# safaad/aim

Hardware: AMD Instinct MI355X
Metric: aligned pairs/sec WFA-adaptive l=100 e=1% (higher is better)
Workload: dtype int16

## Files before the change

aim_amd/csrc/wfa_lane.hpp:

```cpp
#pragma once

#include <utility>

#include "aim_device.hpp"

#ifndef AIM_LANE_MIN_WAVES
#define AIM_LANE_MIN_WAVES 1
#endif
#ifndef AIM_LANE_FULLWAIT
#define AIM_LANE_FULLWAIT 0
#endif
#ifndef AIM_LANE_INTERLEAVE
#define AIM_LANE_INTERLEAVE 2
#endif
#ifndef AIM_LANE_SPREAD_PCT
#define AIM_LANE_SPREAD_PCT 67
#endif
#ifndef AIM_LANE_ASM_ROWS
#define AIM_LANE_ASM_ROWS 1
#endif
#ifndef AIM_LANE_NT_STORE
#define AIM_LANE_NT_STORE 0
#endif
#ifndef AIM_LANE_PACK_X2
#define AIM_LANE_PACK_X2 0
#endif
#ifndef AIM_LANE_STAMPS
#define AIM_LANE_STAMPS 0
#endif
#ifndef AIM_LANE_DIAG
#define AIM_LANE_DIAG 0
#endif
#ifndef AIM_LANE_RES_STAGE
#define AIM_LANE_RES_STAGE 1
#endif
#ifndef AIM_LANE_DMA_AUX
#define AIM_LANE_DMA_AUX 2
#endif
#ifndef AIM_LANE_WGS_PER_CU
#define AIM_LANE_WGS_PER_CU 8
#endif
#if AIM_LANE_STAMPS
#define AIM_STAMP(i) do { unsigned long long t_; __builtin_amdgcn_sched_barrier(0); \
        asm volatile("s_memtime %0\n\ts_waitcnt lgkmcnt(0)" : "=s"(t_) :: "memory"); __builtin_amdgcn_sched_barrier(0); \
        stamp_sum[i] += t_ - stamp_last; stamp_last = t_; } while (0)
#else
#define AIM_STAMP(i) do { } while (0)
#endif

namespace aim {

constexpr int kLaneNull = -16384;

template <int X, int O, int E, int MAXS>
struct WfShape {
    bool present[MAXS + 1];
    bool hasI[MAXS + 1];
    bool hasD[MAXS + 1];
    int lo[MAXS + 1];
    int hi[MAXS + 1];
    int kmin, kmax, maxw;
    constexpr WfShape() : present{}, hasI{}, hasD{}, lo{}, hi{}, kmin(0), kmax(0), maxw(1)
    {
        present[0] = true;
        for (int s = 1; s <= MAXS; ++s) {
            const int ss = s - X, so = s - O - E, se = s - E;
            const bool m_sub_null = ss < 0 || !present[ss];
            const bool m_o_null = so < 0 || !present[so];
            const bool i_e_null = se < 0 || !present[se] || !hasI[se];
            const bool d_e_null = se < 0 || !present[se] || !hasD[se];
            const bool i_out_null = m_o_null && i_e_null;
            const bool d_out_null = m_o_null && d_e_null;
            if (m_sub_null && i_out_null && d_out_null) continue;
            const int sub_lo = m_sub_null ? 1 : lo[ss], sub_hi = m_sub_null ? -1 : hi[ss];
            const int o_lo = m_o_null ? 1 : lo[so], o_hi = m_o_null ? -1 : hi[so];
            const bool e_none = i_e_null && d_e_null;
            const int e_lo = e_none ? 1 : lo[se], e_hi = e_none ? -1 : hi[se];
            int l = sub_lo < o_lo ? sub_lo : o_lo;
            l = (l < e_lo ? l : e_lo) - 1;
            int h = sub_hi > o_hi ? sub_hi : o_hi;
            h = (h > e_hi ? h : e_hi) + 1;
            present[s] = true;
            hasI[s] = !i_out_null;
            hasD[s] = !d_out_null;
            lo[s] = l;
            hi[s] = h;
            if (l < kmin) kmin = l;
            if (h > kmax) kmax = h;
            if (h - l + 1 > maxw) maxw = h - l + 1;
        }
    }
};

template <int X, int O, int E, int MAXS>
struct WfHist {
    int m[MAXS + 1], i[MAXS + 1], d[MAXS + 1];
    int meta, total;
    constexpr WfHist() : m{}, i{}, d{}, meta(0), total(0)
    {
        constexpr WfShape<X, O, E, MAXS> SH{};
        int at = 0;
        for (int s = 0; s <= MAXS; ++s) {
            const int w = SH.present[s] ? SH.hi[s] - SH.lo[s] + 1 : 0;
            m[s] = at; at += w;
            i[s] = at; at += (SH.present[s] && SH.hasI[s]) ? w : 0;
            d[s] = at; at += (SH.present[s] && SH.hasD[s]) ? w : 0;
        }
        meta = at;
        total = at + 3 * (MAXS + 1);
    }
};
enum { LF_PRESENT = 1, LF_MNULL = 2, LF_INULL = 4, LF_DNULL = 8, LF_HASI = 16, LF_HASD = 32 };

template <int NP>
__device__ __forceinline__ int first_stop(const uint32_t (&m)[NP], int v)
{
    const int wi = v >> 4;
    const uint32_t lowmask = ~0u << ((v & 15) * 2);
    int res = NP * 16;
#pragma unroll
    for (int j = NP - 1; j >= 0; --j) {
        uint32_t mj = m[j];
        mj = (j == wi) ? (mj & lowmask) : mj;
        mj = (j < wi) ? 0u : mj;
        const int pos = j * 16 + (__builtin_ctz(mj | 0x80000000u) >> 1);
        res = mj ? pos : res;
    }
    return res;
}

typedef __attribute__((address_space(3))) void *lds_ptr_t;
__device__ __forceinline__ lds_ptr_t lds_at(uint32_t byte_off) { return (lds_ptr_t)(uintptr_t)byte_off; }

template <int... I>
__device__ __forceinline__ void dma_full_pieces(uint32_t lds_off, const char *g_lane, std::integer_sequence<int, I...>)
{
    (__builtin_amdgcn_global_load_lds((const __attribute__((address_space(1))) void *)(g_lane + (I >> 2) * 4096),
                                      lds_at(lds_off + (I >> 2) * 4096), 16, (I & 3) * 1024, AIM_LANE_DMA_AUX), ...);
}

template <int I>
__device__ __forceinline__ void dma_piece(uint32_t lds_off, const char *g_lane)
{
    __builtin_amdgcn_global_load_lds((const __attribute__((address_space(1))) void *)(g_lane + (I >> 2) * 4096),
                                      lds_at(lds_off + (I >> 2) * 4096), 16, (I & 3) * 1024, AIM_LANE_DMA_AUX);
    __builtin_amdgcn_sched_barrier(0);
}

template <int X, int O, int E, int MAXS, int NP, int PCT>
struct LaneSpread {
    int cells, last;
    constexpr LaneSpread() : cells(0), last(0)
    {
        constexpr WfShape<X, O, E, MAXS> SH{};
        for (int s = 0; s <= MAXS; ++s) cells += SH.present[s] ? SH.hi[s] - SH.lo[s] + 1 : 0;
        const int c = (cells * PCT + 99) / 100;
        last = NP + 1 + (c < 1 ? 1 : c);
    }
    constexpr int due(int slot) const { return slot >= last ? NP + 1 : (slot * (NP + 1)) / last; }
};

template <typename F, int... I>
__device__ __forceinline__ void lane_pieces(int from, int to, F &f, std::integer_sequence<int, I...>)
{
    ((I >= from && I < to ? f(std::integral_constant<int, I>{}) : void()), ...);
}
template <int N, typename F>
__device__ __forceinline__ void lane_pieces_from(int first, F &f)
{
    static_assert(N <= 8, "one case per piece");
    switch (first) {
    case 0: if constexpr (0 < N) f(std::integral_constant<int, 0>{}); [[fallthrough]];
    case 1: if constexpr (1 < N) f(std::integral_constant<int, 1>{}); [[fallthrough]];
    case 2: if constexpr (2 < N) f(std::integral_constant<int, 2>{}); [[fallthrough]];
    case 3: if constexpr (3 < N) f(std::integral_constant<int, 3>{}); [[fallthrough]];
    case 4: if constexpr (4 < N) f(std::integral_constant<int, 4>{}); [[fallthrough]];
    case 5: if constexpr (5 < N) f(std::integral_constant<int, 5>{}); [[fallthrough]];
    case 6: if constexpr (6 < N) f(std::integral_constant<int, 6>{}); [[fallthrough]];
    case 7: if constexpr (7 < N) f(std::integral_constant<int, 7>{}); [[fallthrough]];
    default: break;
    }
}

template <int RS, int NCH>
__device__ __forceinline__ void dma_rows(uint32_t lds_off, const char *base, uint32_t pair0, uint32_t n_pairs, int lane)
{
    const char *g = base + (uint64_t)pair0 * RS;
    if (pair0 + kWave <= n_pairs) {
        dma_full_pieces(lds_off, g + (uint32_t)lane * 16u, std::make_integer_sequence<int, NCH>{});
    } else {
        const uint32_t rows = n_pairs - pair0;
        const uint32_t n_chunks = (rows * RS + 15) / 16;
#pragma unroll
        for (int i = 0; i < NCH; ++i) {
            const uint32_t c = i * kWave + lane;
            if (c < n_chunks)
                __builtin_amdgcn_global_load_lds((const __attribute__((address_space(1))) void *)(g + (uint64_t)c * 16),
                                                 lds_at(lds_off + i * kWave * 16), 16, 0, AIM_LANE_DMA_AUX);
        }
    }
}

__device__ __forceinline__ void stage_requests(uint32_t lds_off, const KArgs &a, uint32_t pair0, int lane)
{
    const uint32_t rqb = (a.p.flags & AIM_FLAG_REQ8) ? 8u : 16u;
    const char *g = reinterpret_cast<const char *>(a.req) + (uint64_t)pair0 * rqb;
    if (pair0 + kWave <= a.n_pairs) {
        if ((uint32_t)lane * 16u < kWave * rqb)
            __builtin_amdgcn_global_load_lds((const __attribute__((address_space(1))) void *)(g + (uint64_t)lane * 16),
                                             lds_at(lds_off), 16, 0, 0);
    } else {
        const uint32_t n_dw = (a.n_pairs - pair0) * (rqb / 4u);
#pragma unroll
        for (int i = 0; i < 4; ++i) {
            const uint32_t c = i * kWave + lane;
            if (c < n_dw)
                __builtin_amdgcn_global_load_lds((const __attribute__((address_space(1))) void *)(g + (uint64_t)c * 4),
                                                 lds_at(lds_off + i * kWave * 4), 4, 0, 0);
        }
    }
}

typedef uint32_t lane_u32x4 __attribute__((ext_vector_type(4)));
typedef uint32_t lane_u32x2 __attribute__((ext_vector_type(2)));

struct LaneReqAddr { uint32_t lo, hi; };
__device__ __forceinline__ LaneReqAddr staged_request_addr(uint32_t lds_req_off, const KArgs &a, int lane)
{
    const bool r8 = a.p.flags & AIM_FLAG_REQ8;
    LaneReqAddr q;
    q.lo = lds_req_off + (uint32_t)lane * (r8 ? 8u : 16u);
    q.hi = q.lo + (r8 ? 4u : 12u);
    return q;
}
__device__ __forceinline__ aim_request_t decode_staged_request(const lane_u32x2 &lo, uint32_t hi, const KArgs &a)
{
    aim_request_t r;
    r.padding = 0; r.idx = hi;
    if (a.p.flags & AIM_FLAG_REQ8) { r.pattern_len = (int16_t)(lo.x & 0xffffu); r.text_len = (int16_t)(lo.x >> 16); }
    else { r.pattern_len = (int)lo.x; r.text_len = (int)lo.y; }
    return r;
}

template <int RS, int NP>
__device__ __forceinline__ void read_group(const LaneReqAddr &qa, uint32_t row_addr, lane_u32x2 &q_lo, uint32_t &q_hi,
                                           lane_u32x4 (&P)[NP], lane_u32x4 (&T)[NP])
{
    static_assert(NP == 5 || NP == 7, "READ_SIZE 80 or 112");
#if AIM_LANE_ASM_ROWS
    if constexpr (NP == 7) {
        asm volatile("ds_read_b64 %0, %[qlo]\n\tds_read_b32 %1, %[qhi]\n\t"
                     "ds_read_b128 %2, %[row]\n\tds_read_b128 %3, %[row] offset:16\n\tds_read_b128 %4, %[row] offset:32\n\t"
                     "ds_read_b128 %5, %[row] offset:48\n\tds_read_b128 %6, %[row] offset:64\n\tds_read_b128 %7, %[row] offset:80\n\t"
                     "ds_read_b128 %8, %[row] offset:96\n\t"
                     "ds_read_b128 %9, %[row] offset:%c[tb]\n\tds_read_b128 %10, %[row] offset:%c[tb]+16\n\tds_read_b128 %11, %[row] offset:%c[tb]+32\n\t"
                     "ds_read_b128 %12, %[row] offset:%c[tb]+48\n\tds_read_b128 %13, %[row] offset:%c[tb]+64\n\tds_read_b128 %14, %[row] offset:%c[tb]+80\n\t"
                     "ds_read_b128 %15, %[row] offset:%c[tb]+96\n\t"
                     "s_waitcnt lgkmcnt(0)"
                     : "=&v"(q_lo), "=&v"(q_hi), "=&v"(P[0]), "=&v"(P[1]), "=&v"(P[2]), "=&v"(P[3]), "=&v"(P[4]), "=&v"(P[5]), "=&v"(P[6]),
                       "=&v"(T[0]), "=&v"(T[1]), "=&v"(T[2]), "=&v"(T[3]), "=&v"(T[4]), "=&v"(T[5]), "=&v"(T[6])
                     : [qlo] "v"(qa.lo), [qhi] "v"(qa.hi), [row] "v"(row_addr), [tb] "n"(kWave * RS)
                     : "memory");
    } else {
        asm volatile("ds_read_b64 %0, %[qlo]\n\tds_read_b32 %1, %[qhi]\n\t"
                     "ds_read_b128 %2, %[row]\n\tds_read_b128 %3, %[row] offset:16\n\tds_read_b128 %4, %[row] offset:32\n\t"
                     "ds_read_b128 %5, %[row] offset:48\n\tds_read_b128 %6, %[row] offset:64\n\t"
                     "ds_read_b128 %7, %[row] offset:%c[tb]\n\tds_read_b128 %8, %[row] offset:%c[tb]+16\n\tds_read_b128 %9, %[row] offset:%c[tb]+32\n\t"
                     "ds_read_b128 %10, %[row] offset:%c[tb]+48\n\tds_read_b128 %11, %[row] offset:%c[tb]+64\n\t"
                     "s_waitcnt lgkmcnt(0)"
                     : "=&v"(q_lo), "=&v"(q_hi), "=&v"(P[0]), "=&v"(P[1]), "=&v"(P[2]), "=&v"(P[3]), "=&v"(P[4]),
                       "=&v"(T[0]), "=&v"(T[1]), "=&v"(T[2]), "=&v"(T[3]), "=&v"(T[4])
                     : [qlo] "v"(qa.lo), [qhi] "v"(qa.hi), [row] "v"(row_addr), [tb] "n"(kWave * RS)
                     : "memory");
    }
#else
    typedef const __attribute__((address_space(3))) lane_u32x4 *lds_row_t;
    q_lo = *reinterpret_cast<const __attribute__((address_space(3))) lane_u32x2 *>((uintptr_t)qa.lo);
    q_hi = *reinterpret_cast<const __attribute__((address_space(3))) uint32_t *>((uintptr_t)qa.hi);
#pragma unroll
    for (int j = 0; j < NP; ++j) P[j] = reinterpret_cast<lds_row_t>((uintptr_t)row_addr)[j];
#pragma unroll
    for (int j = 0; j < NP; ++j) T[j] = reinterpret_cast<lds_row_t>((uintptr_t)(row_addr + kWave * RS))[j];
    asm volatile("s_waitcnt lgkmcnt(0)" ::: "memory");
#endif
}

template <int J, bool MASKED, int NP, typename StepF>
__device__ __forceinline__ void pack_step(const lane_u32x4 (&raw)[NP], int len, uint32_t (&out)[NP], uint32_t &bad, StepF &after_step)
{
    const uint32_t a[4] = {raw[J].x, raw[J].y, raw[J].z, raw[J].w};
    uint32_t b[4];
#if AIM_LANE_PACK_X2
#pragma unroll
    for (int i = 0; i < 4; ++i) {
        const uint32_t t2 = a[i] & 0x06060606u;
        const uint32_t rec = __builtin_amdgcn_perm(0x00470054u, 0x00430041u, t2);
        if (MASKED) {
            const int rem = len - 4 * (4 * J + i);
            const uint32_t mask = rem >= 4 ? ~0u : (rem <= 0 ? 0u : ((1u << (8 * rem)) - 1u));
            bad |= (rec ^ a[i]) & mask;
        } else {
            bad = __builtin_amdgcn_sad_u8(rec, a[i], bad);
        }
        b[i] = __builtin_amdgcn_udot4(t2, 0x40100401u, 0u, false);
    }
    out[J] = ((b[0] | (b[1] << 8) | (b[2] << 16)) >> 1) | (b[3] << 23);
#else
#pragma unroll
    for (int i = 0; i < 4; ++i) {
        const uint32_t t = (a[i] >> 1) & 0x03030303u;
        const uint32_t rec = __builtin_amdgcn_perm(0u, 0x47544341u, t);
        if (MASKED) {
            const int rem = len - 4 * (4 * J + i);
            const uint32_t mask = rem >= 4 ? ~0u : (rem <= 0 ? 0u : ((1u << (8 * rem)) - 1u));
            bad |= (rec ^ a[i]) & mask;
        } else {
            bad = __builtin_amdgcn_sad_u8(rec, a[i], bad);
        }
        b[i] = __builtin_amdgcn_udot4(t, 0x40100401u, 0u, false);
    }
    out[J] = b[0] | (b[1] << 8) | (b[2] << 16) | (b[3] << 24);
#endif
    after_step(std::integral_constant<int, J>{});
}
template <bool FAST, int NP, typename StepF, int... J>
__device__ __forceinline__ uint32_t pack_row_seq(const lane_u32x4 (&raw)[NP], int len, uint32_t (&out)[NP], StepF &after_step,
                                                 std::integer_sequence<int, J...>)
{
    uint32_t bad = 0;
    (pack_step<J, (!FAST || J == NP - 1), NP>(raw, len, out, bad, after_step), ...);
    return bad;
}
template <bool FAST, int NP, typename StepF>
__device__ __forceinline__ uint32_t pack_row(const lane_u32x4 (&raw)[NP], int len, uint32_t (&out)[NP], StepF after_step)
{
    return pack_row_seq<FAST, NP>(raw, len, out, after_step, std::make_integer_sequence<int, NP>{});
}

enum : uint32_t { LANE_TODO_COUNT = 0, LANE_TODO_LIST = 16 };

template <int NP>
__device__ __forceinline__ void raw_diag(const lane_u32x4 (&rawP)[NP], const lane_u32x4 (&rawT)[NP], int k, uint32_t (&out)[NP])
{
    uint32_t pw[4 * NP], tw[4 * NP];
#pragma unroll
    for (int j = 0; j < NP; ++j) {
        pw[4 * j] = rawP[j].x; pw[4 * j + 1] = rawP[j].y; pw[4 * j + 2] = rawP[j].z; pw[4 * j + 3] = rawP[j].w;
        tw[4 * j] = rawT[j].x; tw[4 * j + 1] = rawT[j].y; tw[4 * j + 2] = rawT[j].z; tw[4 * j + 3] = rawT[j].w;
    }
#pragma unroll
    for (int j = 0; j < NP; ++j) {
        uint32_t b[4];
#pragma unroll
        for (int i = 0; i < 4; ++i) {
            const int w = 4 * j + i;
            const int o = 4 * w + k;
            const int wi = (o >= 0) ? (o >> 2) : -((-o + 3) >> 2);
            const int sh = o - 4 * wi;
            const uint32_t lo = (wi >= 0 && wi < 4 * NP) ? tw[wi] : 0u;
            const uint32_t hi = (wi + 1 >= 0 && wi + 1 < 4 * NP) ? tw[wi + 1] : 0u;
            const uint32_t ts = sh ? __builtin_amdgcn_alignbyte(hi, lo, (uint32_t)sh) : lo;
            const uint32_t x = pw[w] ^ ts;
            const uint32_t nz = ((((x & 0x7f7f7f7fu) + 0x7f7f7f7fu) | x) >> 7) & 0x01010101u;
            b[i] = __builtin_amdgcn_udot4(nz, 0x40100401u, 0u, false);
        }
        out[j] = b[0] | (b[1] << 8) | (b[2] << 16) | (b[3] << 24);
    }
}



struct LaneNoCell { __device__ __forceinline__ void operator()() const {} };
template <int X, int O, int E, int MAXS, int NP, int KW, bool HIST = false, typename CellF = LaneNoCell>
__device__ __forceinline__ int wfa_scores_dynamic(const uint32_t (&dk)[KW][NP], int plen, int tlen, int ms_run, bool reduce, bool active,
                                                  int16_t *hist = nullptr, CellF on_cell = CellF{})
{
    constexpr WfShape<X, O, E, MAXS> SH{};
    constexpr WfHist<X, O, E, MAXS> HX{};
    bool hasi[MAXS + 1], hasd[MAXS + 1];
    static_assert(KW == SH.kmax - SH.kmin + 1, "diagonal window");
    static_assert(SH.kmax < 16 && SH.kmin > -16, "diagonal shifts are single-word funnel shifts");
    const int ak = tlen - plen;
    int Mv[MAXS + 1][KW], Iv[MAXS + 1][KW], Dv[MAXS + 1][KW];
    int klo[MAXS + 1], khi[MAXS + 1];
    bool pres[MAXS + 1], mnul[MAXS + 1], inul[MAXS + 1], dnul[MAXS + 1];
    int score = MAXS + 1;
    bool done = false;
#pragma unroll
    for (int s = 0; s <= MAXS; ++s) {
        if (!SH.present[s]) {
            pres[s] = false; mnul[s] = inul[s] = dnul[s] = true; klo[s] = 0; khi[s] = -1; hasi[s] = hasd[s] = false;
            if (HIST) { hist[(HX.meta + 3 * s) * kWave] = 0; hist[(HX.meta + 3 * s + 1) * kWave] = -1; hist[(HX.meta + 3 * s + 2) * kWave] = 0; }
            continue;
        }
        if (s == 0) {
            pres[0] = true; mnul[0] = false; inul[0] = dnul[0] = true; klo[0] = khi[0] = 0; hasi[0] = hasd[0] = false;
            Mv[0][-SH.kmin] = 0;
        } else {
            const int ss = s - X, so = s - O - E, se = s - E;
            const bool m_sub_null = ss < 0 || !SH.present[ss] || !pres[ss < 0 ? 0 : ss] || mnul[ss < 0 ? 0 : ss];
            const bool m_o_null = so < 0 || !SH.present[so] || !pres[so < 0 ? 0 : so] || mnul[so < 0 ? 0 : so];
            const bool i_e_null = se < 0 || !SH.present[se] || !pres[se < 0 ? 0 : se] || inul[se < 0 ? 0 : se];
            const bool d_e_null = se < 0 || !SH.present[se] || !pres[se < 0 ? 0 : se] || dnul[se < 0 ? 0 : se];
            const bool i_out_null = m_o_null && i_e_null, d_out_null = m_o_null && d_e_null;
            pres[s] = !(m_sub_null && i_out_null && d_out_null);
            const int sub_lo = m_sub_null ? 1 : klo[ss < 0 ? 0 : ss], sub_hi = m_sub_null ? -1 : khi[ss < 0 ? 0 : ss];
            const int o_lo = m_o_null ? 1 : klo[so < 0 ? 0 : so], o_hi = m_o_null ? -1 : khi[so < 0 ? 0 : so];
            const bool e_none = i_e_null && d_e_null;
            const int e_lo = e_none ? 1 : klo[se < 0 ? 0 : se], e_hi = e_none ? -1 : khi[se < 0 ? 0 : se];
            klo[s] = min(min(sub_lo, o_lo), e_lo) - 1;
            khi[s] = max(max(sub_hi, o_hi), e_hi) + 1;
            mnul[s] = false; inul[s] = i_out_null; dnul[s] = d_out_null;
            hasi[s] = !i_out_null; hasd[s] = !d_out_null;
#pragma unroll
            for (int k = SH.lo[s]; k <= SH.hi[s]; ++k) {
                const int kk = k - SH.kmin;
                const int km1 = kk > 0 ? kk - 1 : 0, kp1 = kk + 1 < KW ? kk + 1 : KW - 1;
                const int sso = so < 0 ? 0 : so, sse = se < 0 ? 0 : se, sss = ss < 0 ? 0 : ss;
                int ins = -10;
                {
                    const int ins_g = (!m_o_null && o_lo <= k - 1 && k - 1 <= o_hi) ? Mv[sso][km1] : kLaneNull;
                    const int ins_i = (!i_e_null && e_lo <= k - 1 && k - 1 <= e_hi) ? Iv[sse][km1] : kLaneNull;
                    const int v = (ins_g == kLaneNull && ins_i == kLaneNull) ? kLaneNull : max(ins_g, ins_i) + 1;
                    ins = i_out_null ? -10 : v;
                    Iv[s][kk] = v;
                    if (HIST && SH.hasI[s]) hist[(HX.i[s] + k - SH.lo[s]) * kWave] = (int16_t)v;
                }
                int del = -10;
                {
                    const int del_g = (!m_o_null && o_lo <= k + 1 && k + 1 <= o_hi) ? Mv[sso][kp1] : kLaneNull;
                    const int del_d = (!d_e_null && e_lo <= k + 1 && k + 1 <= e_hi) ? Dv[sse][kp1] : kLaneNull;
                    const int v = max(del_g, del_d);
                    del = d_out_null ? -10 : v;
                    Dv[s][kk] = v;
                    if (HIST && SH.hasD[s]) hist[(HX.d[s] + k - SH.lo[s]) * kWave] = (int16_t)v;
                }
                int sub = -10;
                if (!m_sub_null) sub = (sub_lo <= k && k <= sub_hi) ? Mv[sss][kk] + 1 : kLaneNull;
                Mv[s][kk] = max(del, max(sub, ins));
            }
        }
#pragma unroll
        for (int k = SH.lo[s]; k <= SH.hi[s]; ++k) {
            const int kk = k - SH.kmin;
            int off = Mv[s][kk];
            const int v = off - k;
            const int limit = min(plen, tlen - k);
            if (off >= 0 && v >= 0 && v < limit) {
                const int stop = min(first_stop<NP>(dk[kk], v), limit);
                off += stop - v;
            }
            Mv[s][kk] = off;
            if (HIST) hist[(HX.m[s] + k - SH.lo[s]) * kWave] = (int16_t)off;
            on_cell();
        }
        if (SH.hi[s] - SH.lo[s] + 1 >= 10) {
            const bool apply = reduce && pres[s] && !mnul[s] && (khi[s] - klo[s] + 1) >= 10;
            int dist[KW];
            int min_distance = max(plen, tlen);
#pragma unroll
            for (int k = SH.lo[s]; k <= SH.hi[s]; ++k) {
                const int kk = k - SH.kmin;
                const int off = Mv[s][kk];
                dist[kk] = max(plen - (off - k), tlen - off);
                if (klo[s] <= k && k <= khi[s]) min_distance = min(min_distance, dist[kk]);
            }
            int kfirst = 0x7fffffff, klast = -0x7fffffff;
#pragma unroll
            for (int k = SH.lo[s]; k <= SH.hi[s]; ++k) {
                const int kk = k - SH.kmin;
                const bool ok = klo[s] <= k && k <= khi[s] && (dist[kk] - min_distance) <= 50;
                kfirst = ok ? min(kfirst, k) : kfirst;
                klast = ok ? max(klast, k) : klast;
            }
            int nklo = klo[s], nkhi = khi[s];
            const int top_limit = min(ak - 1, khi[s]);
            if (klo[s] < top_limit) nklo = min(top_limit, kfirst);
            const int bottom_limit = max(ak + 1, nklo);
            if (khi[s] > bottom_limit) nkhi = max(bottom_limit, klast);
            const bool kill = nklo > nkhi;
            if (apply) {
                mnul[s] = kill; inul[s] = inul[s] || kill; dnul[s] = dnul[s] || kill;
                klo[s] = kill ? klo[s] : nklo;
                khi[s] = kill ? khi[s] : nkhi;
            }
        }
        if (HIST) {
            hist[(HX.meta + 3 * s) * kWave] = (int16_t)klo[s];
            hist[(HX.meta + 3 * s + 1) * kWave] = (int16_t)khi[s];
            hist[(HX.meta + 3 * s + 2) * kWave] = (int16_t)((pres[s] ? LF_PRESENT : 0) | (mnul[s] ? LF_MNULL : 0) | (inul[s] ? LF_INULL : 0) | (dnul[s] ? LF_DNULL : 0) |
                                                            (hasi[s] ? LF_HASI : 0) | (hasd[s] ? LF_HASD : 0));
        }
        {
            int m_end = kLaneNull;
#pragma unroll
            for (int k = SH.lo[s]; k <= SH.hi[s]; ++k) m_end = (k == ak) ? Mv[s][k - SH.kmin] : m_end;
            if (!done && pres[s] && !mnul[s] && klo[s] <= ak && ak <= khi[s] && m_end >= tlen && s <= ms_run) { done = true; score = s; }
        }
        if (__ballot(!done && active) == 0ull) break;
    }
    if (!done) score = ms_run + 1;
    return score;
}

template <int X, int O, int E, int MAXS, int RS, bool BT, bool DYN = false>
__global__ __launch_bounds__(64, DYN ? 2 : AIM_LANE_MIN_WAVES) void wfa_lane_kernel(KArgs a)
{
    constexpr WfShape<X, O, E, MAXS> SH{};
    static_assert(DYN || SH.maxw < 10, "WFA-adaptive reduction could fire: shape needs the dynamic-bounds score loop (DYN)");
    static_assert(!(DYN && BT), "the dynamic-bounds score loop is score-only");
    static_assert(RS % 16 == 0 && (RS / 16) % 2 == 1, "row stride must be an odd number of 16-B slots");
    constexpr int NCH = RS / 16;
    constexpr int NP = RS / 16;
    constexpr int KW = SH.kmax - SH.kmin + 1;
    constexpr bool SPREAD_T = AIM_LANE_INTERLEAVE == 2 && !BT;
    constexpr int NTP = NP + 1;
    constexpr LaneSpread<X, O, E, MAXS, NP, DYN ? 100 : AIM_LANE_SPREAD_PCT> SP{};
    extern __shared__ __attribute__((aligned(16))) char smem[];
    debug_poison_lds(a, smem);
    uint32_t *resL = reinterpret_cast<uint32_t *>(smem) + 2 * kWave * (RS / 4) + kWave * 4;
    const uint32_t lds0 = (uint32_t)(uintptr_t)(lds_ptr_t)smem;
    const uint32_t offP = lds0, offT = lds0 + kWave * RS, offQ = lds0 + 2 * kWave * RS;
    const int lane = threadIdx.x;
    const uint32_t n_groups = (a.n_pairs + kWave - 1) / kWave;
    const int ms_run = a.p.max_score;

    auto next_group = [&](uint32_t it_, uint32_t *g_) -> bool { return xcd_unit(n_groups, it_, g_); };
    uint32_t grp;
    bool have = next_group(0, &grp);
    const bool res8 = a.p.flags & AIM_FLAG_RES8;
    const LaneReqAddr req_addr = staged_request_addr(offQ, a, lane);
    const uint32_t row_addr = offP + (uint32_t)lane * RS;
    if (have) {
        dma_rows<RS, NCH>(offP, a.patterns, grp * kWave, a.n_pairs, lane);
        dma_rows<RS, NCH>(offT, a.texts, grp * kWave, a.n_pairs, lane);
        stage_requests(offQ, a, grp * kWave, lane);
    }
    uint32_t stores_in_flight = 0;
#if AIM_LANE_STAMPS
    unsigned long long stamp_sum[8] = {0, 0, 0, 0, 0, 0, 0, 0}, stamp_last;
    asm volatile("s_memtime %0\n\ts_waitcnt lgkmcnt(0)" : "=s"(stamp_last) :: "memory");
#endif
    for (uint32_t it = 0; have; ++it) {
        const uint32_t pair = grp * kWave + lane;
        const bool active = pair < a.n_pairs;
        const bool full_group = BT && AIM_LANE_RES_STAGE && (grp + 1u) * kWave <= a.n_pairs;
        AIM_STAMP(0);
        if (BT || AIM_LANE_FULLWAIT || stores_in_flight == 0) asm volatile("s_waitcnt vmcnt(0) lgkmcnt(0)" ::: "memory");
        else if (stores_in_flight == 1) asm volatile("s_waitcnt vmcnt(1) lgkmcnt(0)" ::: "memory");
        else asm volatile("s_waitcnt vmcnt(2) lgkmcnt(0)" ::: "memory");
        __builtin_amdgcn_sched_barrier(0);
        AIM_STAMP(1);
        lane_u32x4 rawP[NP], rawT[NP];
        lane_u32x2 rq_lo;
        uint32_t rq_hi;
        __builtin_amdgcn_sched_barrier(0);
        read_group<RS, NP>(req_addr, row_addr, rq_lo, rq_hi, rawP, rawT);
        __builtin_amdgcn_sched_barrier(0);
        const aim_request_t rq = decode_staged_request(rq_lo, rq_hi, a);
        const int plen = active ? rq.pattern_len : 0, tlen = active ? rq.text_len : 0;
        uint32_t ngrp = 0;
        const bool nhave = next_group(it + 1, &ngrp);
        const bool inter = AIM_LANE_INTERLEAVE && !AIM_LANE_DIAG && nhave && (ngrp + 1u) * kWave <= a.n_pairs;
        AIM_STAMP(2);
        if (nhave && !inter) {
            dma_rows<RS, NCH>(offP, a.patterns, ngrp * kWave, a.n_pairs, lane);
            dma_rows<RS, NCH>(offT, a.texts, ngrp * kWave, a.n_pairs, lane);
            stage_requests(offQ, a, ngrp * kWave, lane);
        }
        const char *gP_next = a.patterns + (uint64_t)ngrp * (kWave * RS) + (uint32_t)lane * 16u;
        const char *gT_next = a.texts + (uint64_t)ngrp * (kWave * RS) + (uint32_t)lane * 16u;
        __builtin_amdgcn_sched_barrier(0);
        AIM_STAMP(3);
#if AIM_LANE_DIAG == 1 || AIM_LANE_DIAG == 4
        {
            uint32_t x = 0;
#pragma unroll
            for (int j = 0; j < NP; ++j) x ^= rawP[j].x ^ rawP[j].y ^ rawP[j].z ^ rawP[j].w ^ rawT[j].x ^ rawT[j].y ^ rawT[j].z ^ rawT[j].w;
            if (active && (AIM_LANE_DIAG == 1 || x == 0x12345678u)) {
                aim_result_t r;
                r.max_operations = plen + tlen; r.begin_offset = 0; r.end_offset = 0; r.score = (int)x; r.status = 0; r.idx = rq.idx;
                store_result(a, pair, r);
            }
            stores_in_flight = AIM_LANE_DIAG == 1 ? (res8 ? 1u : 2u) : 0u;
            have = nhave; grp = ngrp;
            continue;
        }
#endif
        const int minlen = active ? min(plen, tlen) : 0x7fffffff;
        const int min_len_wave = __builtin_amdgcn_readfirstlane(wave_min_i32(minlen));
        uint32_t P[NP], T[NP];
        uint32_t bad;
        auto t_piece = [&](auto I) __attribute__((always_inline)) {
            constexpr int i = decltype(I)::value;
            if constexpr (i < NP) dma_piece<i>(offT, gT_next);
            else { stage_requests(offQ, a, ngrp * kWave, lane); __builtin_amdgcn_sched_barrier(0); }
        };
        auto pack_both = [&](auto FAST, auto INTER) __attribute__((always_inline)) {
            constexpr bool fast = decltype(FAST)::value, with_dma = decltype(INTER)::value;
            bad = pack_row<fast, NP>(rawP, plen, P, [&](auto J) { if (with_dma) dma_piece<decltype(J)::value>(offP, gP_next); });
            bad |= pack_row<fast, NP>(rawT, tlen, T, [&](auto J) {
                constexpr int j = decltype(J)::value;
                if (with_dma && SPREAD_T) lane_pieces(SP.due(j), SP.due(j + 1), t_piece, std::make_integer_sequence<int, NTP>{});
                else if (with_dma) dma_piece<j>(offT, gT_next);
            });
            if (with_dma && !SPREAD_T) stage_requests(offQ, a, ngrp * kWave, lane);
        };
        const bool fast = min_len_wave >= 16 * (NP - 1);
        if (fast && inter) pack_both(std::true_type{}, std::true_type{});
        else if (fast) pack_both(std::true_type{}, std::false_type{});
        else if (inter) pack_both(std::false_type{}, std::true_type{});
        else pack_both(std::false_type{}, std::false_type{});

        AIM_STAMP(4);
#if AIM_LANE_DIAG == 2
        {
            uint32_t x = bad;
#pragma unroll
            for (int j = 0; j < NP; ++j) x ^= P[j] ^ T[j];
            if (active) {
                aim_result_t r;
                r.max_operations = plen + tlen; r.begin_offset = 0; r.end_offset = 0; r.score = (int)x; r.status = 0; r.idx = rq.idx;
                store_result(a, pair, r);
            }
            stores_in_flight = res8 ? 1u : 2u;
            have = nhave; grp = ngrp;
            continue;
        }
#endif
        const int ak = tlen - plen;
        int Mv[MAXS + 1][KW], Iv[MAXS + 1][KW], Dv[MAXS + 1][KW];
        int score = MAXS + 1;
        bool done = false;
        auto score_phase = [&](auto SPREAD) __attribute__((always_inline)) {
        constexpr bool spread = decltype(SPREAD)::value;
        int slot = NP, t_out = SP.due(NP);
        auto at_slot = [&]() __attribute__((always_inline)) {
            if constexpr (spread) {
                ++slot;
                lane_pieces(t_out, SP.due(slot), t_piece, std::make_integer_sequence<int, NTP>{});
                t_out = SP.due(slot);
            }
        };
        uint32_t dk[KW][NP];
        if (__ballot(active && bad != 0u) != 0ull) {
#pragma unroll
            for (int kk = 0; kk < KW; ++kk) raw_diag<NP>(rawP, rawT, SH.kmin + kk, dk[kk]);
        } else {
#pragma unroll
            for (int kk = 0; kk < KW; ++kk) {
                const int k = SH.kmin + kk;
#pragma unroll
                for (int j = 0; j < NP; ++j) {
                    uint32_t ts;
                    if (k == 0) ts = T[j];
                    else if (k > 0) ts = __builtin_amdgcn_alignbit(j + 1 < NP ? T[j + 1] : 0u, T[j], 2 * k);
                    else ts = __builtin_amdgcn_alignbit(T[j], j > 0 ? T[j - 1] : 0u, 32 + 2 * k);
                    dk[kk][j] = P[j] ^ ts;
                }
            }
        }
        at_slot();

        if constexpr (DYN) {
            score = wfa_scores_dynamic<X, O, E, MAXS, NP, KW, false, decltype(at_slot)>(dk, plen, tlen, ms_run, (a.p.flags & AIM_FLAG_REDUCE) != 0, active,
                                                                                        nullptr, at_slot);
            done = score <= ms_run;
        } else {
#pragma unroll
        for (int s = 0; s <= MAXS; ++s) {
            if (!SH.present[s]) continue;
            if (s > 0) {
                const int ss = s - X, so = s - O - E, se = s - E;
                const bool sub_ok = ss >= 0 && SH.present[ss];
                const bool o_ok = so >= 0 && SH.present[so];
                const bool ie_ok = se >= 0 && SH.present[se] && SH.hasI[se];
                const bool de_ok = se >= 0 && SH.present[se] && SH.hasD[se];
#pragma unroll
                for (int k = SH.lo[s]; k <= SH.hi[s]; ++k) {
                    const int kk = k - SH.kmin;
                    const int km1 = kk > 0 ? kk - 1 : 0, kp1 = kk + 1 < KW ? kk + 1 : KW - 1;
                    int ins = -10;
                    if (SH.hasI[s]) {
                        const int ins_g = (o_ok && SH.lo[so] <= k - 1 && k - 1 <= SH.hi[so]) ? Mv[so][km1] : kLaneNull;
                        const int ins_i = (ie_ok && SH.lo[se] <= k - 1 && k - 1 <= SH.hi[se]) ? Iv[se][km1] : kLaneNull;
                        ins = (ins_g == kLaneNull && ins_i == kLaneNull) ? kLaneNull : max(ins_g, ins_i) + 1;
                        Iv[s][kk] = ins;
                    }
                    int del = -10;
                    if (SH.hasD[s]) {
                        const int del_g = (o_ok && SH.lo[so] <= k + 1 && k + 1 <= SH.hi[so]) ? Mv[so][kp1] : kLaneNull;
                        const int del_d = (de_ok && SH.lo[se] <= k + 1 && k + 1 <= SH.hi[se]) ? Dv[se][kp1] : kLaneNull;
                        del = max(del_g, del_d);
                        Dv[s][kk] = del;
                    }
                    int sub = -10;
                    if (sub_ok) sub = (SH.lo[ss] <= k && k <= SH.hi[ss]) ? Mv[ss][kk] + 1 : kLaneNull;
                    Mv[s][kk] = max(del, max(sub, ins));
                }
            } else {
                Mv[0][-SH.kmin] = 0;
            }
            int m_end = kLaneNull;
            bool end_in_range = false;
#pragma unroll
            for (int k = SH.lo[s]; k <= SH.hi[s]; ++k) {
                const int kk = k - SH.kmin;
                int off = Mv[s][kk];
                const int v = off - k;
                const int limit = min(plen, tlen - k);
                if (off >= 0 && v >= 0 && v < limit) {
                    const int stop = min(first_stop<NP>(dk[kk], v), limit);
                    off += stop - v;
                }
                Mv[s][kk] = off;
                if (k == ak) { m_end = off; end_in_range = true; }
                at_slot();
            }
            if (!done && end_in_range && m_end >= tlen && s <= ms_run) { done = true; score = s; }
            if (__ballot(!done && active) == 0ull) break;
        }
        if (!done) score = ms_run + 1;
        }
        if constexpr (spread) lane_pieces_from<NTP>(t_out, t_piece);
        };
        if (SPREAD_T && inter) score_phase(std::true_type{});
        else score_phase(std::false_type{});
        AIM_STAMP(5);

        int begin_offset = plen + tlen - 1;
        int status = AIM_PAIR_OK;
        const int gap_len = done ? max(0, score - O) / E : 0;
        const int w_lo = BT ? wave_min_i32(active ? max(0, (done ? min(plen, tlen) - gap_len : plen + tlen - 1)) >> 4 : (1 << 20)) : 0;
        const int w_hi = BT ? -wave_min_i32(active ? -((plen + tlen + 15) >> 4) : 0) : 0;
        if (BT && active) {
            char *ops = a.ops + (uint64_t)pair * (2 * RS);
            uint4 *orow = reinterpret_cast<uint4 *>(ops);
            const uint4 mm = make_uint4(0x4D4D4D4Du, 0x4D4D4D4Du, 0x4D4D4D4Du, 0x4D4D4D4Du);
#pragma unroll
            for (int j = 0; j < (2 * RS) / 16; ++j)
                if (j >= w_lo && j < w_hi) orow[j] = mm;
            if (done) {
                constexpr int kNone = (int)0x80000000;
                auto getM = [&](int s_, int k_) {
                    int r = kNone;
#pragma unroll
                    for (int s2 = 0; s2 <= MAXS; ++s2)
                        if (SH.present[s2])
#pragma unroll
                            for (int k2 = SH.lo[s2]; k2 <= SH.hi[s2]; ++k2) r = (s_ == s2 && k_ == k2) ? Mv[s2][k2 - SH.kmin] : r;
                    return r;
                };
                auto getI = [&](int s_, int k_) {
                    int r = kNone;
#pragma unroll
                    for (int s2 = 0; s2 <= MAXS; ++s2)
                        if (SH.present[s2] && SH.hasI[s2])
#pragma unroll
                            for (int k2 = SH.lo[s2]; k2 <= SH.hi[s2]; ++k2) r = (s_ == s2 && k_ == k2) ? Iv[s2][k2 - SH.kmin] : r;
                    return r;
                };
                auto getD = [&](int s_, int k_) {
                    int r = kNone;
#pragma unroll
                    for (int s2 = 0; s2 <= MAXS; ++s2)
                        if (SH.present[s2] && SH.hasD[s2])
#pragma unroll
                            for (int k2 = SH.lo[s2]; k2 <= SH.hi[s2]; ++k2) r = (s_ == s2 && k_ == k2) ? Dv[s2][k2 - SH.kmin] : r;
                    return r;
                };
                auto valid_loc = [&](int kk_, int off_) {
                    const int v_ = off_ - kk_, h_ = off_;
                    return v_ > 0 && v_ <= plen && h_ > 0 && h_ <= tlen;
                };
                auto put = [&](char ch) {
                    if (begin_offset >= 0 && begin_offset < 2 * RS) ops[begin_offset] = ch;
                    --begin_offset;
                };
                enum { BT_M = 0, BT_I = 1, BT_D = 2 };
                int sc = score, k = ak;
                int offset = getM(sc, k);
                bool valid = valid_loc(k, offset);
                int bt = BT_M;
                int v = offset - k, h = offset;
                while (v > 0 && h > 0 && sc > 0) {
                    if (!valid) {
                        valid = valid_loc(k, offset);
                        if (valid) {
                            if (k < ak) for (int i = k; i < ak; ++i) put('I');
                            else if (k > ak) for (int i = ak; i < k; ++i) put('D');
                        }
                    }
                    const int s_o = sc - (O + E), s_e = sc - E, s_x = sc - X;
                    int del_ext = kLaneNull, del_open = kLaneNull, ins_ext = kLaneNull, ins_open = kLaneNull, misms = kLaneNull;
                    if (bt != BT_I) {
                        const int a1 = getD(s_e, k + 1), a2 = getM(s_o, k + 1);
                        if (a1 != kNone) del_ext = a1;
                        if (a2 != kNone) del_open = a2;
                    }
                    if (bt != BT_D) {
                        const int a1 = getI(s_e, k - 1), a2 = getM(s_o, k - 1);
                        if (a1 != kNone) ins_ext = a1 + 1;
                        if (a2 != kNone) ins_open = a2 + 1;
                    }
                    if (bt == BT_M) {
                        const int a1 = getM(s_x, k);
                        if (a1 != kNone) misms = a1 + 1;
                    }
                    const int max_all = max(misms, max(max(ins_ext, ins_open), max(del_ext, del_open)));
                    if (bt == BT_M) {
                        const int num_matches = offset - max_all;
                        if (num_matches > 0) begin_offset -= num_matches;
                        offset = max_all;
                        v = offset - k;
                        h = offset;
                        if (v <= 0 || h <= 0) break;
                    }
                    char op;
                    if (max_all == del_ext) { op = 'D'; sc = s_e; ++k; bt = BT_D; }
                    else if (max_all == del_open) { op = 'D'; sc = s_o; ++k; bt = BT_M; }
                    else if (max_all == ins_ext) { op = 'I'; sc = s_e; --k; --offset; bt = BT_I; }
                    else if (max_all == ins_open) { op = 'I'; sc = s_o; --k; --offset; bt = BT_M; }
                    else if (max_all == misms) { op = 'X'; sc = s_x; --offset; }
                    else { status = AIM_PAIR_WFA_NO_LINK; break; }
                    if (valid) put(op);
                    v = offset - k;
                    h = offset;
                }
                if (status == AIM_PAIR_OK) {
                    if (sc == 0) {
                        if (offset > 0) begin_offset -= offset;
                    } else {
                        for (; v > 0; --v) put('D');
                        for (; h > 0; --h) put('I');
                    }
                    ++begin_offset;
                }
            }
        }
        if (active) {
            {
                aim_result_t r;
                r.max_operations = plen + tlen;
                r.begin_offset = begin_offset;
                r.end_offset = plen + tlen;
                r.score = score;
                r.status = status;
                r.idx = rq.idx;
#if AIM_LANE_DIAG == 3
                if (score == 0x12345678)
#endif
#if AIM_LANE_RES_STAGE
                if (full_group) {
                    uint32_t *rl = resL + lane * 6;
                    rl[0] = (uint32_t)r.max_operations; rl[1] = (uint32_t)r.begin_offset; rl[2] = (uint32_t)r.end_offset;
                    rl[3] = (uint32_t)r.score; rl[4] = (uint32_t)r.status; rl[5] = (uint32_t)r.idx;
                } else
#endif
                if (BT) {
                    store_result(a, pair, r);
                } else if (res8) {
                    typedef uint32_t aim_u32x2 __attribute__((ext_vector_type(2)));
                    aim_u32x2 v2; v2.x = r.idx; v2.y = (uint32_t)r.score;
                    aim_u32x2 *dst2 = reinterpret_cast<aim_u32x2 *>(reinterpret_cast<aim_result8_t *>(a.res) + pair);
                    if (AIM_LANE_NT_STORE) __builtin_nontemporal_store(v2, dst2); else *dst2 = v2;
                } else {
                    uint32_t *dst = reinterpret_cast<uint32_t *>(a.res + pair);
                    *reinterpret_cast<uint4 *>(dst) = make_uint4((uint32_t)r.max_operations, (uint32_t)r.begin_offset, (uint32_t)r.end_offset, (uint32_t)r.score);
                    *reinterpret_cast<uint2 *>(dst + 4) = make_uint2((uint32_t)r.status, r.idx);
                }
            }
        }
        stores_in_flight = (BT || AIM_LANE_DIAG == 3) ? 0u : (res8 ? 1u : 2u);
#if AIM_LANE_RES_STAGE
        if (full_group) {
            typedef uint32_t aim_u32x4 __attribute__((ext_vector_type(4)));
            asm volatile("s_waitcnt lgkmcnt(0)" ::: "memory");
            const aim_u32x4 *src = reinterpret_cast<const aim_u32x4 *>(resL);
            aim_u32x4 *dst = reinterpret_cast<aim_u32x4 *>(a.res + (size_t)grp * kWave);
            const aim_u32x4 c0 = src[lane];
            __builtin_nontemporal_store(c0, dst + lane);
            if (lane < 32) { const aim_u32x4 c1 = src[64 + lane]; __builtin_nontemporal_store(c1, dst + 64 + lane); }
        }
#endif
        have = nhave;
        grp = ngrp;
        AIM_STAMP(6);
    }
#if AIM_LANE_STAMPS
    if (lane == 0) {
        unsigned long long *dbg = reinterpret_cast<unsigned long long *>(a.scratch + a.scratch_per_wave) + (size_t)blockIdx.x * 8;
        for (int i = 0; i < 8; ++i) dbg[i] = stamp_sum[i];
    }
#endif
}


constexpr int kLaneDynMaxScore = 10;

#define AIM_LANE_COST_SETS(F) F(3, 4, 1, 5) F(4, 6, 2, 8) F(2, 3, 1, 4) F(5, 4, 2, 6)

inline int wfa_lane_static_max_score(const aim_params_t &p)
{
#define AIM_LANE_COST_TEST(X, O, E, MS) if (p.mismatch == X && p.gap_o == O && p.gap_e == E) return MS;
    AIM_LANE_COST_SETS(AIM_LANE_COST_TEST)
#undef AIM_LANE_COST_TEST
    return -1;
}

inline bool wfa_lane_supported(const aim_params_t &p, bool allow_dynamic = true)
{
    if (p.algo != AIM_ALGO_WFA) return false;
    const int ms = wfa_lane_static_max_score(p);
    if (ms < 0) return false;
    if (p.read_size != 80 && p.read_size != 112) return false;
    if (p.max_score <= ms) return true;
    if (p.mismatch != 3 || p.gap_o != 4 || p.gap_e != 1) return false;
    return allow_dynamic && p.max_score <= kLaneDynMaxScore && !(p.flags & AIM_FLAG_BACKTRACE);
}

inline size_t wfa_lane_todo_bytes(uint32_t n_pairs) { return ((size_t)(LANE_TODO_LIST + n_pairs) * 4 + 255) & ~(size_t)255; }

inline void wfa_lane_plan(const aim_params_t &p, uint32_t n_pairs, const Knobs &kn, uint32_t *grid, uint32_t *block, size_t *lds)
{
    const uint32_t n_groups = (n_pairs + kWave - 1) / kWave;
    uint32_t g = resident_grid(kn, AIM_LANE_WGS_PER_CU);
    const uint32_t need = ((n_groups + 7u) / 8u) * 8u;
    if (g > need) g = need < 8u ? 8u : need;
    *grid = g;
    *block = kWave;
    *lds = (size_t)2 * kWave * p.read_size + kWave * 16 + ((p.flags & AIM_FLAG_BACKTRACE) ? kWave * sizeof(aim_result_t) : 0);
}

#ifdef AIM_TU_WFA_LANE
void wfa_lane_launch(const aim_params_t &p, uint32_t grid, uint32_t block, size_t lds, const KArgs &ka, hipStream_t s)
{
    (void)block;
    const bool bt = p.flags & AIM_FLAG_BACKTRACE;
    if (p.max_score > wfa_lane_static_max_score(p)) {
        if (p.read_size == 80) hipLaunchKernelGGL((wfa_lane_kernel<3, 4, 1, kLaneDynMaxScore, 80, false, true>), dim3(grid), dim3(kWave), lds, s, ka);
        else hipLaunchKernelGGL((wfa_lane_kernel<3, 4, 1, kLaneDynMaxScore, 112, false, true>), dim3(grid), dim3(kWave), lds, s, ka);
        return;
    }
#define AIM_LANE_LAUNCH(X, O, E, MS)                                                                                             \
    if (p.mismatch == X && p.gap_o == O && p.gap_e == E) {                                                                       \
        if (p.read_size == 80) {                                                                                                 \
            if (bt) hipLaunchKernelGGL((wfa_lane_kernel<X, O, E, MS, 80, true>), dim3(grid), dim3(kWave), lds, s, ka);           \
            else hipLaunchKernelGGL((wfa_lane_kernel<X, O, E, MS, 80, false>), dim3(grid), dim3(kWave), lds, s, ka);             \
        } else if (p.read_size == 112) {                                                                                         \
            if (bt) hipLaunchKernelGGL((wfa_lane_kernel<X, O, E, MS, 112, true>), dim3(grid), dim3(kWave), lds, s, ka);          \
            else hipLaunchKernelGGL((wfa_lane_kernel<X, O, E, MS, 112, false>), dim3(grid), dim3(kWave), lds, s, ka);            \
        }                                                                                                                        \
        return;                                                                                                                  \
    }
    AIM_LANE_COST_SETS(AIM_LANE_LAUNCH)
#undef AIM_LANE_LAUNCH
}
#else
void wfa_lane_launch(const aim_params_t &p, uint32_t grid, uint32_t block, size_t lds, const KArgs &ka, hipStream_t s);
#endif

}
```

Baseline: 23.37 billion.

## Buffer 8-byte results in an LDS ring and flush as wide sc1 stores

For the non-backtrace RES8 output path, per-pair 8-byte results are written into an LDS ring of up to 8 group slots. When the ring fills, or at kernel end, it is drained with 16-byte global stores that cover two groups per instruction, using a stride that assumes groups are assigned to blocks in an XCD-interleaved order. Stores now use inline asm with the sc1 cache-policy bit, and since the ring path sets stores_in_flight to 0, the next iteration waits on vmcnt(0). The aim is to replace many small scattered stores with fewer wide ones and cut store-wait stalls, at the cost of extra LDS per workgroup, LDS write waits, and reliance on the group-to-block mapping.

```diff
diff --git a/aim_amd/csrc/wfa_lane.hpp b/aim_amd/csrc/wfa_lane.hpp
--- a/aim_amd/csrc/wfa_lane.hpp
+++ b/aim_amd/csrc/wfa_lane.hpp
@@ -1,5 +1,6 @@
 #pragma once
 
+#include <cassert>
 #include <utility>
 
 #include "aim_device.hpp"
@@ -22,6 +23,15 @@
 #ifndef AIM_LANE_NT_STORE
 #define AIM_LANE_NT_STORE 0
 #endif
+#ifndef AIM_LANE_RES_RING
+#define AIM_LANE_RES_RING 8
+#endif
+#ifndef AIM_LANE_STORE_X4
+#define AIM_LANE_STORE_X4 0
+#endif
+#ifndef AIM_LANE_STORE_SC1
+#define AIM_LANE_STORE_SC1 1
+#endif
 #ifndef AIM_LANE_PACK_X2
 #define AIM_LANE_PACK_X2 0
 #endif
@@ -40,6 +50,7 @@
 #ifndef AIM_LANE_WGS_PER_CU
 #define AIM_LANE_WGS_PER_CU 8
 #endif
+#define AIM_LANE_RING_SLOTS ((AIM_LANE_DIAG == 3 || AIM_LANE_DIAG == 4) ? 0 : AIM_LANE_RES_RING)
 #if AIM_LANE_STAMPS
 #define AIM_STAMP(i) do { unsigned long long t_; __builtin_amdgcn_sched_barrier(0); \
         asm volatile("s_memtime %0\n\ts_waitcnt lgkmcnt(0)" : "=s"(t_) :: "memory"); __builtin_amdgcn_sched_barrier(0); \
@@ -285,6 +296,49 @@
 #endif
 }
 
+__device__ __forceinline__ void lane_store8(void *dst, const lane_u32x2 &v)
+{
+#if AIM_LANE_STORE_SC1
+    asm volatile("global_store_dwordx2 %0, %1, off sc1" :: "v"(dst), "v"(v) : "memory");
+#else
+    if (AIM_LANE_NT_STORE) __builtin_nontemporal_store(v, reinterpret_cast<lane_u32x2 *>(dst)); else *reinterpret_cast<lane_u32x2 *>(dst) = v;
+#endif
+}
+__device__ __forceinline__ void lane_store16(void *dst, const lane_u32x4 &v)
+{
+#if AIM_LANE_STORE_SC1
+    asm volatile("global_store_dwordx4 %0, %1, off sc1\n\ts_nop 1" :: "v"(dst), "v"(v) : "memory");
+#else
+    if (AIM_LANE_NT_STORE) __builtin_nontemporal_store(v, reinterpret_cast<lane_u32x4 *>(dst)); else *reinterpret_cast<lane_u32x4 *>(dst) = v;
+#endif
+}
+
+__device__ __forceinline__ void ring_put(uint32_t lds_addr, uint32_t idx, uint32_t score)
+{
+    lane_u32x2 v; v.x = idx; v.y = score;
+    asm volatile("ds_write_b64 %0, %1\n\ts_waitcnt lgkmcnt(0)" :: "v"(lds_addr), "v"(v) : "memory");
+}
+template <int K, bool FULL>
+__device__ __forceinline__ void ring_flush(uint32_t lds_lane, char *dst_lane, uint64_t step, uint32_t count, int lane)
+{
+    static_assert(K == 4 || K == 8, "two slots per store instruction");
+    lane_u32x4 v[K / 2];
+    if constexpr (K == 8) {
+        asm volatile("ds_read_b128 %0, %4\n\tds_read_b128 %1, %4 offset:1024\n\tds_read_b128 %2, %4 offset:2048\n\tds_read_b128 %3, %4 offset:3072\n\t"
+                     "s_waitcnt lgkmcnt(0)"
+                     : "=&v"(v[0]), "=&v"(v[1]), "=&v"(v[2]), "=&v"(v[3]) : "v"(lds_lane) : "memory");
+    } else {
+        asm volatile("ds_read_b128 %0, %2\n\tds_read_b128 %1, %2 offset:1024\n\ts_waitcnt lgkmcnt(0)"
+                     : "=&v"(v[0]), "=&v"(v[1]) : "v"(lds_lane) : "memory");
+    }
+#pragma unroll
+    for (int q = 0; q < K / 2; ++q) {
+        if (FULL || 2u * q + ((uint32_t)lane >> 5) < count) {
+            lane_store16(dst_lane + q * step, v[q]);
+        }
+    }
+}
+
 template <int J, bool MASKED, int NP, typename StepF>
 __device__ __forceinline__ void pack_step(const lane_u32x4 (&raw)[NP], int len, uint32_t (&out)[NP], uint32_t &bad, StepF &after_step)
 {
@@ -537,6 +591,16 @@
         stage_requests(offQ, a, grp * kWave, lane);
     }
     uint32_t stores_in_flight = 0;
+    constexpr int RING = BT ? 0 : AIM_LANE_RING_SLOTS;
+    const uint32_t offR = offQ + kWave * 16;
+    const uint32_t bpx = gridDim.x >> 3;
+    uint32_t ring_fill = 0, ring_grp0 = 0;
+    auto ring_drain = [&](auto FULL, uint32_t count) __attribute__((always_inline)) {
+        if constexpr (RING > 0) {
+            char *dst = reinterpret_cast<char *>(a.res) + ((uint64_t)ring_grp0 + ((uint32_t)lane >> 5) * bpx) * (kWave * 8u) + ((uint32_t)lane & 31u) * 16u;
+            ring_flush<RING, decltype(FULL)::value>(offR + (uint32_t)lane * 16u, dst, (uint64_t)bpx * (2u * kWave * 8u), count, lane);
+        }
+    };
 #if AIM_LANE_STAMPS
     unsigned long long stamp_sum[8] = {0, 0, 0, 0, 0, 0, 0, 0}, stamp_last;
     asm volatile("s_memtime %0\n\ts_waitcnt lgkmcnt(0)" : "=s"(stamp_last) :: "memory");
@@ -557,6 +621,39 @@
         __builtin_amdgcn_sched_barrier(0);
         read_group<RS, NP>(req_addr, row_addr, rq_lo, rq_hi, rawP, rawT);
         __builtin_amdgcn_sched_barrier(0);
+        if constexpr (RING > 0) {
+            if (ring_fill == RING) {
+                ring_drain(std::true_type{}, RING);
+                ring_fill = 0;
+            }
+            __builtin_amdgcn_sched_barrier(0);
+        }
+        auto store_res8 = [&](uint32_t idx, uint32_t sc, bool on) __attribute__((always_inline)) {
+            if (RING > 0 && (grp + 1u) * kWave <= a.n_pairs) {
+                if (ring_fill == 0) ring_grp0 = grp;
+                ring_put(offR + ring_fill * (kWave * 8u) + (uint32_t)lane * 8u, idx, sc);
+                ++ring_fill;
+                stores_in_flight = 0;
+                return;
+            }
+            aim_result8_t *dst = reinterpret_cast<aim_result8_t *>(a.res) + pair;
+            lane_u32x2 v2; v2.x = idx; v2.y = sc;
+#if AIM_LANE_STORE_X4
+            const uint32_t nidx = (uint32_t)__builtin_amdgcn_update_dpp(0, (int)idx, 0xF5, 0xf, 0xf, false);
+            const uint32_t nsc = (uint32_t)__builtin_amdgcn_update_dpp(0, (int)sc, 0xF5, 0xf, 0xf, false);
+            if (!(lane & 1)) {
+                if (on && pair + 1u < a.n_pairs) {
+                    lane_u32x4 v4; v4.x = idx; v4.y = sc; v4.z = nidx; v4.w = nsc;
+                    lane_store16(dst, v4);
+                } else if (on) {
+                    lane_store8(dst, v2);
+                }
+            }
+#else
+            if (on) lane_store8(dst, v2);
+#endif
+            stores_in_flight = 1;
+        };
         const aim_request_t rq = decode_staged_request(rq_lo, rq_hi, a);
         const int plen = active ? rq.pattern_len : 0, tlen = active ? rq.text_len : 0;
         uint32_t ngrp = 0;
@@ -577,12 +674,16 @@
             uint32_t x = 0;
 #pragma unroll
             for (int j = 0; j < NP; ++j) x ^= rawP[j].x ^ rawP[j].y ^ rawP[j].z ^ rawP[j].w ^ rawT[j].x ^ rawT[j].y ^ rawT[j].z ^ rawT[j].w;
-            if (active && (AIM_LANE_DIAG == 1 || x == 0x12345678u)) {
-                aim_result_t r;
-                r.max_operations = plen + tlen; r.begin_offset = 0; r.end_offset = 0; r.score = (int)x; r.status = 0; r.idx = rq.idx;
-                store_result(a, pair, r);
-            }
-            stores_in_flight = AIM_LANE_DIAG == 1 ? (res8 ? 1u : 2u) : 0u;
+            if (AIM_LANE_DIAG == 1 && res8) {
+                store_res8(rq.idx, x, active);
+            } else {
+                if (active && (AIM_LANE_DIAG == 1 || x == 0x12345678u)) {
+                    aim_result_t r;
+                    r.max_operations = plen + tlen; r.begin_offset = 0; r.end_offset = 0; r.score = (int)x; r.status = 0; r.idx = rq.idx;
+                    store_result(a, pair, r);
+                }
+                stores_in_flight = AIM_LANE_DIAG == 1 ? 2u : 0u;
+            }
             have = nhave; grp = ngrp;
             continue;
         }
@@ -838,7 +939,13 @@
                 }
             }
         }
-        if (active) {
+        if (!BT && res8) {
+            bool on = active;
+#if AIM_LANE_DIAG == 3
+            on = on && score == 0x12345678;
+#endif
+            store_res8(rq.idx, (uint32_t)score, on);
+        } else if (active) {
             {
                 aim_result_t r;
                 r.max_operations = plen + tlen;
@@ -859,19 +966,22 @@
 #endif
                 if (BT) {
                     store_result(a, pair, r);
-                } else if (res8) {
-                    typedef uint32_t aim_u32x2 __attribute__((ext_vector_type(2)));
-                    aim_u32x2 v2; v2.x = r.idx; v2.y = (uint32_t)r.score;
-                    aim_u32x2 *dst2 = reinterpret_cast<aim_u32x2 *>(reinterpret_cast<aim_result8_t *>(a.res) + pair);
-                    if (AIM_LANE_NT_STORE) __builtin_nontemporal_store(v2, dst2); else *dst2 = v2;
                 } else {
                     uint32_t *dst = reinterpret_cast<uint32_t *>(a.res + pair);
+#if AIM_LANE_STORE_SC1 >= 2
+                    lane_u32x4 v4; v4.x = (uint32_t)r.max_operations; v4.y = (uint32_t)r.begin_offset; v4.z = (uint32_t)r.end_offset; v4.w = (uint32_t)r.score;
+                    lane_u32x2 v2; v2.x = (uint32_t)r.status; v2.y = r.idx;
+                    lane_store16(dst, v4);
+                    lane_store8(dst + 4, v2);
+#else
                     *reinterpret_cast<uint4 *>(dst) = make_uint4((uint32_t)r.max_operations, (uint32_t)r.begin_offset, (uint32_t)r.end_offset, (uint32_t)r.score);
                     *reinterpret_cast<uint2 *>(dst + 4) = make_uint2((uint32_t)r.status, r.idx);
+#endif
                 }
             }
         }
-        stores_in_flight = (BT || AIM_LANE_DIAG == 3) ? 0u : (res8 ? 1u : 2u);
+        if (BT || AIM_LANE_DIAG == 3) stores_in_flight = 0;
+        else if (!res8) stores_in_flight = 2;
 #if AIM_LANE_RES_STAGE
         if (full_group) {
             typedef uint32_t aim_u32x4 __attribute__((ext_vector_type(4)));
@@ -887,6 +997,7 @@
         grp = ngrp;
         AIM_STAMP(6);
     }
+    if (ring_fill) ring_drain(std::false_type{}, ring_fill);
 #if AIM_LANE_STAMPS
     if (lane == 0) {
         unsigned long long *dbg = reinterpret_cast<unsigned long long *>(a.scratch + a.scratch_per_wave) + (size_t)blockIdx.x * 8;
@@ -930,6 +1041,9 @@
     *grid = g;
     *block = kWave;
     *lds = (size_t)2 * kWave * p.read_size + kWave * 16 + ((p.flags & AIM_FLAG_BACKTRACE) ? kWave * sizeof(aim_result_t) : 0);
+    static_assert(AIM_LANE_RING_SLOTS == 0 || AIM_LANE_RING_SLOTS == 4 || AIM_LANE_RING_SLOTS == 8, "AIM_LANE_RES_RING: 0, 4 or 8");
+    if (!(p.flags & AIM_FLAG_BACKTRACE) && (p.flags & AIM_FLAG_RES8)) *lds += (size_t)AIM_LANE_RING_SLOTS * kWave * 8;
+    assert(lds_workgroups_per_cu(*lds) >= AIM_LANE_WGS_PER_CU);
 }
 
 #ifdef AIM_TU_WFA_LANE
```

After: 24.61 billion (median of 6 runs). 1.05x the previous value.
